# data61/gossamer

Measured on AMD Instinct MI355X. Metric: M k-mers/s (canonical, counted) at k=25, 150 bp reads, higher is better.
Workload: dtype u64

## Files before the change

### gossamer_amd/csrc/fused_path.hpp

```cpp
#pragma once

enum { kFusedDeclined = 0, kFusedDone = 1, kFusedNeedFull = 2, kFusedGoOn = -1, kFusedAgain = -2 };
constexpr uint32_t kFusedGrid = 256 * GOSS_E1_OCC;
#ifndef GOSS_FUSED_NKEYS2
#define GOSS_FUSED_NKEYS2 14
#endif
#ifndef GOSS_FUSED_GRID2
#define GOSS_FUSED_GRID2 512
#endif
constexpr uint32_t kFusedGrid2 = GOSS_FUSED_GRID2;
constexpr double kValidSlackA = 1.06, kValidSlackB = 1.17;
constexpr uint64_t kValidSizingMin = 640u << 20;

struct FusedForm {
    enum Table {
        kSmall,
        kBig,
        kWide,
        k96,
        kRem32
    };
    Table table = kSmall;
    uint32_t segbits = kSegBits;
    bool msd = false;
// ... 497 lines not shown
    if (n == 0) return kFusedDeclined;
    if (n > ch.ka_slots || n > ch.kb_slots) return ch.decline("more keys than the buffers hold");
    const bool narrow = form.rem32() && form.narrow;
    uint64_t tiles = 0, sum = 0;
    const uint64_t tile_keys = narrow ? (uint64_t)(form.r32_bits == 9 ? Sub32N<9>::kTileSlots : Sub32N<10>::kTileSlots)
                             : form.rem32() ? (uint64_t)kSub32Tile : form.msd ? (uint64_t)SubCfg<K>::kTile : (uint64_t)SortCfg<K, false>::kTile;
    for (int d = 0; d < 256; ++d)
    {
        gt->cnt[d] = hp->cursors[d * kCursorStride];
        gt->tile_first[d] = tiles;
        tiles += (gt->cnt[d] + tile_keys - 1) / tile_keys;
        sum += gt->cnt[d];
    }
    gt->tile_first[256] = tiles;
    const uint64_t n_slots = narrow ? n / 3 * 2 : n;
    const uint64_t B = 1ULL << br.blk_log2;
    if (sum < n_slots || sum > n_slots + 8 + (uint64_t)br.grid * 256 * (2 * B + 8))
        throw StatusError{GOSS_ERR_HIP, "fused extraction: bucket counts do not add up"};
    HIP_TRY(hipMemcpyAsync(dgt, gt, sizeof(GapTable), hipMemcpyHostToDevice, c->stream));
    out->n = n; out->tiles = tiles; out->windows = hp->windows;
    return kFusedGoOn;
}

struct FusedLookback { LookbackCtl* ctl; LookbackCtl* hctl; };

inline int count_rem32(const FusedChunk<Key1>& ch, FusedForm form, const Sub32Regions& sub, const FirstLevelResult& fl, const GapTable* dgt,
                       FusedLookback lb, Run* r)
{
    goss_gpu_ctx* c = ch.c;
    Key1* ka = ch.ka; Key1* kb = ch.kb;
    const uint64_t n = fl.n, tiles = fl.tiles;
    const uint32_t r32_regions = form.r32_regions(), r32_bits = form.r32_bits, r32_split = form.r32_split, rbits32 = form.rbits32;
    const uint32_t sqbit32 = c->len - 1;
    const bool narrow = form.narrow, squeeze = form.squeeze;
    SubTable32* dsub = (SubTable32*)c->arena.temp(sizeof(SubTable32));
    unsigned long long* cur2 = (unsigned long long*)c->arena.temp((uint64_t)r32_regions * 4);
    uint64_t* seg_beg = (uint64_t*)c->arena.temp((uint64_t)r32_regions * 8);
    uint64_t* seg_end = (uint64_t*)c->arena.temp((uint64_t)r32_regions * 8);
    Tile32* tdesc = (Tile32*)c->arena.temp(std::max<uint64_t>(tiles, 1) * sizeof(Tile32));
    HIP_TRY(hipMemcpyAsync(dsub->start, sub.start.data(), (uint64_t)r32_regions * 8, hipMemcpyHostToDevice, c->stream));
    HIP_TRY(hipMemcpyAsync(dsub->cap, sub.cap.data(), (uint64_t)r32_regions * 4, hipMemcpyHostToDevice, c->stream));
    HIP_TRY(hipMemsetAsync(cur2, 0, (uint64_t)r32_regions * 4, c->stream));
    if (narrow && r32_bits == 9)
        hipLaunchKernelGGL(HIP_KERNEL_NAME(tiles32_kernel<Sub32N<9>::kTileSlots>), dim3(grid_for(tiles, 256)), dim3(256), 0, c->stream,
                           dgt, tdesc, (uint32_t)tiles);
    else if (narrow)
        hipLaunchKernelGGL(HIP_KERNEL_NAME(tiles32_kernel<Sub32N<10>::kTileSlots>), dim3(grid_for(tiles, 256)), dim3(256), 0, c->stream,
                           dgt, tdesc, (uint32_t)tiles);
    else
        hipLaunchKernelGGL(HIP_KERNEL_NAME(tiles32_kernel<kSub32Tile>), dim3(grid_for(tiles, 256)), dim3(256), 0, c->stream,
                           dgt, tdesc, (uint32_t)tiles);
    {
        PhaseTimer t(c, GOSS_T_SCATTER, n);
        const dim3 g2((uint32_t)((tiles + 7) / 8 * 8));
#define GOSS_LAUNCH_S32N(SQ, B2, NRW)                                                                                    \
    hipLaunchKernelGGL(HIP_KERNEL_NAME(subpart32_kernel<SQ, B2, NRW>), g2, dim3(kTB), 0, c->stream, (const Key1*)ka, (uint32_t*)kb, rbits32, \
                       sqbit32, cur2, (const Tile32*)tdesc, (uint32_t)tiles, (const SubTable32*)dsub, lb.ctl)
#define GOSS_LAUNCH_S32(SQ, B2) do { if (narrow) GOSS_LAUNCH_S32N(SQ, B2, true); else GOSS_LAUNCH_S32N(SQ, B2, false); } while (0)
        if (squeeze) GOSS_LAUNCH_S32(true, 9);
        else if (r32_bits == 9) GOSS_LAUNCH_S32(false, 9);
        else GOSS_LAUNCH_S32(false, 10);
#undef GOSS_LAUNCH_S32
#undef GOSS_LAUNCH_S32N
        t.stop();
    }
    hipLaunchKernelGGL(sub_bounds32_kernel, dim3(r32_regions / 256), dim3(256), 0, c->stream, (const SubTable32*)dsub,
                       (const uint32_t*)cur2, r32_regions, seg_beg, seg_end);
    HIP_TRY(hipMemcpyAsync(lb.hctl, lb.ctl, sizeof(LookbackCtl), hipMemcpyDeviceToHost, c->stream));
    HIP_TRY(hipStreamSynchronize(c->stream));
    if (lb.hctl->error) { c->fused_overflows++; return ch.decline("a 32-bit sub-region overflowed"); }
    ch.lap("second level (32-bit remainders)");
    const uint32_t* rems = (const uint32_t*)kb;
    Key1* spare32 = ka;
    uint32_t nseg32 = r32_regions;
    if (r32_split)
    {
        nseg32 = r32_regions << r32_split;
        uint64_t* sub_beg = (uint64_t*)c->arena.temp((uint64_t)nseg32 * 8);
        uint64_t* sub_end = (uint64_t*)c->arena.temp((uint64_t)nseg32 * 8);
        {
            PhaseTimer t(c, GOSS_T_SCATTER, n);
            hipLaunchKernelGGL(subsplit32_kernel, unit_grid(r32_regions), dim3(kTB), 0, c->stream, (const uint32_t*)kb, (uint32_t*)ka,
                               (const uint64_t*)seg_beg, (const uint64_t*)seg_end, rbits32 - (squeeze ? 1u : 0u), r32_split, sub_beg, sub_end);
            t.stop();
        }
        check_launch("third-level split kernel");
        seg_beg = sub_beg; seg_end = sub_end;
        rems = (const uint32_t*)ka;
        spare32 = kb;
        ch.lap("third level (sub-segments)");
    }
    int rc;
    for (;;)
    {
        rc = segment_reduce32(c, rems, spare32, n, r, seg_beg, seg_end, form.r32_slots, squeeze, rbits32, sqbit32, nseg32, r32_split);
        if (rc != 1 || form.r32_slots >= 16384 || c->rem32_slots) break;
        c->segment_retries++;
        form = form.larger_r32_table();
    }
    if (rc != 0)
    {
        c->segment_retries++;
        if (rc == 1 && r32_split < (uint32_t)kSub32SplitMax) c->rem32_split_min = r32_split + 1;
        else c->rem32 = false;
        if (c->debug) std::fprintf(stderr, "libgossgpu: fused path: 32-bit form with %u + %u bits overflowed (%d), redoing the chunk %s\n", r32_bits, r32_split, rc,
                                   c->rem32 ? "with more sub-segments" : "in the 8-byte form");
        return kFusedAgain;
// ... 241 lines not shown
```

### gossamer_amd/csrc/goss_gpu.hip

```cpp
#include "../../include/goss_gpu.h"

#include <hip/hip_runtime.h>
#include <dlfcn.h>

#include <algorithm>
#include <chrono>
#include <cmath>
#include <cstdio>
#include <cstdlib>
#include <cstring>
#include <functional>
#include <map>
#include <mutex>
#include <string>
#include <system_error>
#include <thread>
#include <vector>

#include "goss_kernels.hpp"
#include "goss_reader.hpp"

using namespace goss;

namespace {
// ... 66 lines not shown
    double est_scale = 1.0;
    uint32_t order_bits = 0;
    bool ordered_tiles = false;
    uint32_t lookback_failures = 0;
    uint64_t emit_estimate = 0;
    bool has_emit_estimate = false;
    struct Pending { hipEvent_t ev; void (*fn)(void*); void* user; };
    std::vector<Pending> pending;
    uint64_t flush_wait_us = 0, flush_count_us = 0, flushes = 0;
    struct PackedSrc { bool on = false; const uint32_t* codes = nullptr; const uint16_t* bad = nullptr; } pk;
    bool stage_pk[2] = {false, false};
    uint8_t* stage_buf[2] = {nullptr, nullptr};
    int stage_cur = 0;
    hipStream_t copy_stream = nullptr;
    std::thread bg;
    int bg_status = GOSS_OK;
    std::string bg_error;
    std::vector<hipEvent_t> pend_pool;
    uint8_t* stage = nullptr;
    uint64_t stage_cap = 0, stage_fill = 0;
    bool mute_timing = false;
    uint32_t segment_retries = 0;
    uint32_t extract_hist_shift = 0xFFFFFFFFu;
    bool extract_rep = false;
    uint32_t rep_chunks = 0;
    bool graph_rep = true;
    int canon_l1 = 1;
    bool more_follows = false;
    uint64_t more_starts = 0;
    uint64_t expect_bases = 0;
    int space_choice = -1;
    uint32_t canon_chunks = 0;
    bool fused = true;
    uint64_t fused_min = 32u << 20;
    uint32_t fused_overflows = 0;
    uint32_t valid_sized_chunks = 0;
    uint32_t valid_resizes = 0;
    uint64_t dump_lo = 0;
    bool dump_live = false;
    uint64_t budget_limit = 0;
    uint32_t arena_grows = 0;
    uint64_t arena_ms = 0;
    std::thread arena_thread;
    int arena_status = GOSS_OK;
    std::string arena_error;
    uint32_t seg_merges = 0;
    uint32_t hash_merges = 0;
    uint64_t hash_merge_min = 1u << 20;
    bool fused_msd = true;
    uint32_t fused_msd_chunks = 0;
    bool rem32 = true;
    int rem32_slots = 0;
    uint32_t narrow_capg = 656;
    bool narrow = true;
    uint32_t r32_small_max = 0;
    bool overflow_by_sort = true;
    uint64_t overflow_units = 0;
    uint32_t rem32_chunks = 0;
    uint32_t narrow_chunks = 0;
    uint64_t assemble_us = 0;
    uint64_t ds_blocks_ranges = 0, ds_blocks_own = 0;
    uint32_t pk_fused_chunks = 0;
    uint32_t pk_unpacked_chunks = 0;
    uint32_t rem32_bits_min = 0;
    uint32_t rem32_bits_last = 0;
    uint32_t rem32_split_min = 0;
    uint32_t rem32_split_last = 0;
    uint32_t fused_chunks = 0;
    bool debug = false;
    double fused_capscale = 1.0;
    uint32_t blk_log2_max = 0;
    bool no_fast32 = false;
    bool table96 = true;
    uint32_t table96_chunks = 0;
    bool wide_table = true;
    bool big_table = true;
    int big_rounds_min = 0;
    uint32_t big_table_chunks = 0;
    uint32_t wide_table_chunks = 0;
    bool rec_mode = false;
    uint32_t rec_chunks = 0;
    bool deferred = false;
    uint8_t* grp_send = nullptr;
    uint64_t grp_send_cap = 0;
    uint8_t* grp_inbox = nullptr;
    uint64_t grp_inbox_cap = 0;
    hipStream_t xstream = nullptr;
    double valid_frac = 1.0;
    bool size_by_valid = true;
    uint64_t budget = 0;
    hipStream_t stream = nullptr;
    bool own_stream = false;
    std::string last_error;
    Arena arena;
    std::vector<Run> runs;
    std::vector<BigMap> big_maps;
    BigMap res_big;
    uint64_t windows = 0, keys_total = 0;
    bool finished = false, emitted = false;
    bool broken = false;
    double grp_count_ms = 0;
    void* res_keys = nullptr;
    uint32_t* res_counts = nullptr;
    uint64_t M = 0;
    void* tips_keys = nullptr;
    uint32_t* tips_counts = nullptr;
// ... 2274 lines not shown
    {
        case GOSS_OK: return "ok";
        case GOSS_ERR_INVALID_ARG: return "invalid argument";
        case GOSS_ERR_NO_DEVICE: return "no usable gfx950 HIP device";
        case GOSS_ERR_OOM: return "out of memory (HBM budget)";
        case GOSS_ERR_HIP: return "HIP runtime error";
        case GOSS_ERR_STATE: return "call out of order";
        case GOSS_ERR_K_RANGE: return "unable to build a graph with that k";
        case GOSS_ERR_COUNT_OVERFLOW: return "a key count does not fit 32 bits";
        case GOSS_ERR_TOO_LARGE: return "SparseArray high bits do not fit 64 bits";
        case GOSS_ERR_BUFFER: return "a buffer of the caller is too small";
        default: return "unknown status";
    }
}

const char* goss_gpu_last_error(const goss_gpu_ctx* ctx) { return ctx ? ctx->last_error.c_str() : ""; }

uint32_t goss_gpu_abi_version(void) { return kAbiVersion; }

int goss_gpu_create(goss_gpu_ctx** out, int device, uint32_t k, int mode, uint64_t hbm_budget, void* stream)
{
    if (!out) return GOSS_ERR_INVALID_ARG;
    *out = nullptr;
    if (mode != GOSS_MODE_KMER_SET && mode != GOSS_MODE_GRAPH) return GOSS_ERR_INVALID_ARG;
    if (k == 0) return GOSS_ERR_K_RANGE;
    if (mode == GOSS_MODE_KMER_SET && k > 63) return GOSS_ERR_K_RANGE;
    if (mode == GOSS_MODE_GRAPH && k > 62) return GOSS_ERR_K_RANGE;
    int ndev = 0;
    if (hipGetDeviceCount(&ndev) != hipSuccess || ndev <= 0 || device < 0 || device >= ndev) return GOSS_ERR_NO_DEVICE;
    hipDeviceProp_t prop;
    if (hipGetDeviceProperties(&prop, device) != hipSuccess) return GOSS_ERR_NO_DEVICE;
    if (std::strncmp(prop.gcnArchName, "gfx950", 6) != 0) return GOSS_ERR_NO_DEVICE;
    goss_gpu_ctx* c = new (std::nothrow) goss_gpu_ctx();
    if (!c) return GOSS_ERR_OOM;
    c->device = device; c->k = k; c->mode = mode;
    c->len = mode == GOSS_MODE_GRAPH ? k + 1 : k;
    c->words = (2 * c->len <= 62) ? 1 : 2;
    c->budget = hbm_budget;
    { const char* e = std::getenv("GOSS_GPU_NO_LOOKBACK"); if (e && *e == '1') c->lookback = false; }
    { const char* e = std::getenv("GOSS_GPU_ORDERED_TILES"); if (e && *e == '1') c->ordered_tiles = true; }
    { const char* e = std::getenv("GOSS_GPU_EST_SCALE"); if (e && std::atof(e) > 0) c->est_scale = std::atof(e); }
    { const char* e = std::getenv("GOSS_GPU_ORDER_BITS"); if (e && std::atoi(e) >= 16 && std::atoi(e) <= 24) c->order_bits = (uint32_t)std::atoi(e); }
    { const char* e = std::getenv("GOSS_GPU_NO_FUSED"); if (e && *e == '1') c->fused = false; }
    { const char* e = std::getenv("GOSS_GPU_NO_MSD"); if (e && *e == '1') c->fused_msd = false; }
    { const char* e = std::getenv("GOSS_GPU_NO_GRAPH_REP"); if (e && *e && *e != '0') c->graph_rep = false; }
    { const char* e = std::getenv("GOSS_GPU_CANON_L1"); if (e && *e >= '0' && *e <= '2') c->canon_l1 = *e - '0'; }
    { const char* e = std::getenv("GOSS_GPU_NO_REM32"); if (e && *e && *e != '0') c->rem32 = false; }
    { const char* e = std::getenv("GOSS_GPU_REM32_BITS"); if (e && std::atoi(e) >= 9 && std::atoi(e) <= 10) c->rem32_bits_min = (uint32_t)std::atoi(e); }
    { const char* e = std::getenv("GOSS_GPU_REM32_SPLIT"); if (e && std::atoi(e) >= 0 && std::atoi(e) <= 4) c->rem32_split_min = (uint32_t)std::atoi(e); }
    { const char* e = std::getenv("GOSS_GPU_REM32_SLOTS"); if (e && (std::atoi(e) == 2048 || std::atoi(e) == 4096 || std::atoi(e) == 8192 || std::atoi(e) == 16384)) c->rem32_slots = std::atoi(e); }
    { const char* e = std::getenv("GOSS_GPU_NARROW"); if (e) c->narrow = std::atoi(e) != 0; }
    { const char* e = std::getenv("GOSS_GPU_OVERFLOW_BY_SORT"); if (e) c->overflow_by_sort = std::atoi(e) != 0; }
    { const char* e = std::getenv("GOSS_GPU_NARROW_CAPG"); if (e && std::atoi(e) > 0) c->narrow_capg = (uint32_t)std::atoi(e); }
    { const char* e = std::getenv("GOSS_GPU_R32_SMALL_MAX"); if (e) c->r32_small_max = (uint32_t)std::atoi(e); }
    { const char* e = std::getenv("GOSS_GPU_NO_BIG_TABLE"); if (e && *e && *e != '0') c->big_table = false; }
    { const char* e = std::getenv("GOSS_GPU_HASH_MERGE_MIN"); if (e && *e) c->hash_merge_min = std::strtoull(e, nullptr, 10); }
    { const char* e = std::getenv("GOSS_GPU_BLK_LOG2"); if (e && *e) c->blk_log2_max = (uint32_t)std::atoi(e); }
    { const char* e = std::getenv("GOSS_GPU_NO_FAST32"); if (e && *e == '1') c->no_fast32 = true; }
    { const char* e = std::getenv("GOSS_GPU_NO_TABLE96"); if (e && *e && *e != '0') c->table96 = false; }
    { const char* e = std::getenv("GOSS_GPU_NO_WIDE_TABLE"); if (e && *e && *e != '0') c->wide_table = false; }
    { const char* e = std::getenv("GOSS_GPU_BIG_ROUNDS_MIN"); if (e && *e) c->big_rounds_min = std::min(3, std::max(0, std::atoi(e))); }
    { const char* e = std::getenv("GOSS_GPU_NO_VALID_SIZING"); if (e && *e && *e != '0') c->size_by_valid = false; }
    { const char* e = std::getenv("GOSS_GPU_FUSED_MIN"); if (e && *e) c->fused_min = std::strtoull(e, nullptr, 10); }
    { const char* e = std::getenv("GOSS_GPU_FUSED_CAPSCALE"); if (e && *e) c->fused_capscale = std::atof(e); }
    { const char* e = std::getenv("GOSS_GPU_DEBUG"); if (e && *e == '1') c->debug = true; }
    int rc = guarded(c, [&]() {
        if (stream) { c->stream = (hipStream_t)stream; c->own_stream = false; }
        else { HIP_TRY(hipStreamCreateWithFlags(&c->stream, hipStreamNonBlocking)); c->own_stream = true; }
        HIP_TRY(hipMalloc((void**)&c->d_ctr, sizeof(ExtractCounters)));
        HIP_TRY(hipMalloc((void**)&c->d_flags, 16));
        HIP_TRY(hipMemsetAsync(c->d_flags, 0, 16, c->stream));
        HIP_TRY(hipHostMalloc(&c->h_pinned, 256, hipHostMallocDefault));
    });
    if (rc != GOSS_OK) { goss_gpu_destroy(c); return rc == GOSS_ERR_HIP ? GOSS_ERR_NO_DEVICE : rc; }
    *out = c;
    return GOSS_OK;
}

int goss_gpu_prepare(goss_gpu_ctx* c)
{
    if (!c) return GOSS_ERR_INVALID_ARG;
    if (c->arena.base || c->arena_thread.joinable()) return GOSS_OK;
    c->arena_status = GOSS_OK;
    c->arena_thread = std::thread([c]() {
        try
        {
            HIP_TRY(hipSetDevice(c->device));
            map_arena(c);
        }
        catch (const HipError& e) { c->arena_status = GOSS_ERR_HIP; c->arena_error = std::string(e.what) + ": " + hipGetErrorString(e.e); }
        catch (const StatusError& e) { c->arena_status = e.status; c->arena_error = e.msg; }
    });
    return GOSS_OK;
}

void goss_gpu_destroy(goss_gpu_ctx* c)
{
    if (!c) return;
    if (c->arena_thread.joinable()) c->arena_thread.join();
    (void)hipSetDevice(c->device);
    if (c->bg.joinable()) c->bg.join();
    if (c->copy_stream) (void)hipStreamSynchronize(c->copy_stream);
    if (c->stream) (void)hipStreamSynchronize(c->stream);
    for (auto& pd : c->pending) { if (pd.fn) pd.fn(pd.user); (void)hipEventDestroy(pd.ev); }
    for (auto e : c->pend_pool) (void)hipEventDestroy(e);
    for (auto*& b : c->stage_buf) if (b) (void)hipFree(b);
// ... 2523 lines not shown
```

### gossamer_amd/csrc/kernels_count.hpp

```cpp
#pragma once
#include <type_traits>

#include <hip/hip_runtime.h>
#include <stdint.h>

#include "goss_key.hpp"
#include "kernels_partition.hpp"

namespace goss {


constexpr int kSegBits = 16;
constexpr int kSegBitsMax = 24;
constexpr int kSegSlots = 4096;
constexpr int kSegLimit = 3072;
constexpr int kSegSlots2 = 2048;
constexpr int kSegLimit2 = 1536;

template <class K>
__global__ void seg_bounds_kernel(const K* __restrict__ keys, uint64_t n, uint32_t shift, uint32_t nseg,
                                  uint64_t* __restrict__ seg_off)
{
    uint32_t s = blockIdx.x * blockDim.x + threadIdx.x;
    if (s > nseg) return;
// ... 686 lines not shown
                    else if (key != mk && eo < 16u)
                    {
                        const uint32_t slot = 4 * bk + (eo >> 2);
                        const uint32_t old = atomicCAS(&tkey[slot], mk, key);
                        if (old == mk) { atomicAdd(&ndist, 1u); hit = slot; }
                        else if (old == key) hit = slot;
                    }
                    else
                    {
                        if (st == 0) { bk = second_of(f, bk); st = 1; }
                        else bk = (bk + 1) & (NB - 1u);
                        if (++moves > NB) { *vovf = 1; busy = false; pd = 0; }
                    }
                    if (hit != ~0u) { atomicAdd(&tcnt[hit], 1u); busy = false; }
                }
            }
        };
        const bool whole = i0 + (uint32_t)NT * kVec <= nfull && (i0 != 0 || head == 0);
        if (whole)
        {
#pragma unroll
            for (int u = 0; u < kVec; ++u)
            {
                const uint32_t left = four_keys(cur[u], 0xFu, std::true_type{});
                if (__builtin_expect(__ballot(left != 0) != 0, 0)) slow_keys(cur[u], left);
            }
        }
        else
        {
#pragma unroll
            for (int u = 0; u < kVec; ++u)
            {
                const uint32_t i = i0 + (uint32_t)u * NT + tid;
                const uint32_t have = i < nvec ? (n - 4u * i >= 4u ? 4u : n - 4u * i) : 0u;
                uint32_t live = (1u << have) - 1u;
                if (i == 0) live &= ~((1u << head) - 1u);
                const uint32_t left = four_keys(cur[u], live, std::false_type{});
                if (__ballot(left != 0)) slow_keys(cur[u], left);
            }
        }
        GOSS_STAMP(2);
        if (*(lds_vu32)&ndist > (uint32_t)kLimit) *vovf = 1;
        if (*vovf) break;
        GOSS_STAMP(3);
    }
    __syncthreads();
    GOSS_STAMP(4);
    if (ovf)
    {
        if (tid == 0) { atomicOr(&so->overflow, 1u); seg_pos[s] = 0; seg_cnt[s] = kSegOverflowed; }
        return;
    }

    constexpr int kPer = SLOTS / NT;
    constexpr int kBins = SLOTS / 4, kBinsPer = kBins / NT, kBinBits = BB;
    __shared__ uint32_t bins[kBins];
    __shared__ uint32_t sh_scan2[NT / 64 + 1];
    __shared__ uint32_t big;
    unsigned long long ck[kPer];
#pragma unroll
    for (int j = 0; j < kPer; ++j) ck[j] = ((unsigned long long)tcnt[tid * kPer + j] << 32) | tkey[tid * kPer + j];
    for (uint32_t i = tid; i < kBins; i += NT) bins[i] = 0;
    if (tid == 0) big = 0;
    __syncthreads();
    const uint32_t rem_bits = rbits - (SQ ? 1u : 0u);
    const uint32_t bsh = rem_bits > (uint32_t)kBinBits + split_bits ? rem_bits - split_bits - kBinBits : 0;
    uint32_t rnk[kPer];
#pragma unroll
    for (int j = 0; j < kPer; ++j)
        if ((ck[j] >> 32) != 0) rnk[j] = atomicAdd(&bins[((uint32_t)ck[j] >> bsh) & (kBins - 1)], 1u);
    __syncthreads();
    uint32_t bn[kBinsPer], bs[kBinsPer], mine = 0;
#pragma unroll
    for (int q = 0; q < kBinsPer; ++q) { bn[q] = bins[tid * kBinsPer + q]; mine += bn[q]; }
    uint32_t tot_occ;
    uint32_t at = block_excl_scan_n<uint32_t, NT / 64>(mine, sh_scan2, &tot_occ);
    lds_vu32 vbig = (lds_vu32)&big;
#pragma unroll
    for (int q = 0; q < kBinsPer; ++q)
    {
        bs[q] = at; bins[tid * kBinsPer + q] = at; at += bn[q];
        if (bn[q] > 24) *vbig = 1;
    }
    __syncthreads();
#pragma unroll
    for (int j = 0; j < kPer; ++j)
        if ((ck[j] >> 32) != 0)
            tab[bins[((uint32_t)ck[j] >> bsh) & (kBins - 1)] + rnk[j]] = (ck[j] << 32) | (ck[j] >> 32);
    __syncthreads();
    if (!big)
    {
#pragma unroll
        for (int q = 0; q < kBinsPer; ++q)
            for (uint32_t i = 1; i < bn[q]; ++i)
            {
                const unsigned long long kk = tab[bs[q] + i];
                uint32_t j = i;
                while (j > 0 && tab[bs[q] + j - 1] > kk) { tab[bs[q] + j] = tab[bs[q] + j - 1]; --j; }
                tab[bs[q] + j] = kk;
            }
        __syncthreads();
    }
    else
    {
        uint32_t nsort = 512;
        while (nsort < tot_occ) nsort <<= 1;
        for (uint32_t i = tot_occ + tid; i < nsort; i += NT) tab[i] = ~0ULL;
        __syncthreads();
        for (uint32_t k2 = 2; k2 <= nsort; k2 <<= 1)
            for (uint32_t j = k2 >> 1; j > 0; j >>= 1)
            {
                for (uint32_t t = tid; t < nsort / 2; t += NT)
                {
                    const uint32_t i = 2 * t - (t & (j - 1));
                    const uint32_t p = i + j;
                    const bool up = (i & k2) == 0;
                    const unsigned long long a = tab[i], c2 = tab[p];
                    if ((a > c2) == up) { tab[i] = c2; tab[p] = a; }
                }
                __syncthreads();
            }
    }
    GOSS_STAMP(5);
    const uint32_t d = ndist;
    if (tid == 0)
    {
        sh_base = atomicAdd(&so->cursor, (unsigned long long)d);
        if (sh_base + d > so->stage_cap) { atomicOr(&so->overflow, 2u); sh_base = ~0ULL; }
        seg_pos[s] = sh_base;
        seg_cnt[s] = d;
    }
    __syncthreads();
    const uint64_t ob = sh_base;
    if (ob == ~0ULL) return;
    const uint64_t prefix = (uint64_t)(s >> split_bits) << rbits;
    for (uint32_t i = tid; i < d; i += NT)
    {
        const unsigned long long v = tab[i];
        stage_keys[ob + i].lo = prefix | rem32_unpack<SQ>((uint32_t)(v >> 32), sqbit);
        stage_counts[ob + i] = (uint32_t)v;
    }
    GOSS_STAMP(6);
#if defined(GOSS_STAMPS)
    if (tid == 0)
    {
        for (int i = 0; i < 7; ++i) atomicAdd(&so->stamps[i], st_acc[i]);
        atomicAdd(&so->stamps[7], 1ULL);
    }
#endif
#undef GOSS_STAMP
}

constexpr uint32_t kSegLock = 0x80000000u;

template <int NT, int SLOTS>
__device__ __forceinline__ void seg_hash_reduce2_body(const Key2* __restrict__ keys, const uint64_t* __restrict__ seg_off,
                                                      const uint64_t* __restrict__ seg_end, SegOut* __restrict__ so, uint64_t* __restrict__ seg_pos,
                                                      uint64_t* __restrict__ seg_cnt,
                                                      Key2* __restrict__ stage_keys, uint32_t* __restrict__ stage_counts,
                                                      uint32_t rem_bits_all, uint32_t round_bits)
{
    constexpr int kLimit = SLOTS / 4 * 3;
    constexpr bool kPow2 = (SLOTS & (SLOTS - 1)) == 0;
    constexpr int kSlotBits = SLOTS == 2048 ? 11 : SLOTS == 4096 ? 12 : SLOTS == 6144 ? 13 : -1;
    static_assert(kSlotBits > 0 && SLOTS % NT == 0, "table size");
    auto next_slot = [](uint32_t a) { return kPow2 ? ((a + 1) & (uint32_t)(SLOTS - 1)) : (a + 1 == (uint32_t)SLOTS ? 0u : a + 1); };
    __shared__ unsigned long long tlo[SLOTS];
    __shared__ unsigned long long thi[SLOTS];
    __shared__ uint32_t st[SLOTS];
    __shared__ uint32_t ndist;
    __shared__ uint32_t ovf;
    __shared__ unsigned long long sh_base;
    const uint32_t s = unit_block(), tid = threadIdx.x;
    const uint32_t sseg = s >> round_bits, rnd = s & ((1u << round_bits) - 1u);
    const uint32_t rsh = rem_bits_all - round_bits;
    const uint64_t b = seg_off[sseg], e = seg_end[sseg];
    if (b == e)
    {
        if (tid == 0) { seg_pos[s] = 0; seg_cnt[s] = 0; }
        return;
    }
// ... 632 lines not shown
```

### gossamer_amd/csrc/kernels_partition.hpp

```cpp
#pragma once

#include <hip/hip_runtime.h>
#include <stdint.h>

#include "goss_key.hpp"
#include "kernels_common.hpp"

namespace goss {


#ifndef GOSS_SORT_ITEMS1
#define GOSS_SORT_ITEMS1 32
#endif
#ifndef GOSS_SORT_ITEMS2
#define GOSS_SORT_ITEMS2 16
#endif
#ifndef GOSS_LB_BATCH
#define GOSS_LB_BATCH 1
#endif
template <class K> struct SubCfg {
    static constexpr int kItems = sizeof(K) == 8 ? 22 : 11;
    static constexpr int kTile = 256 * kItems;
};

// ... 486 lines not shown

struct Tile32 { unsigned long long base; uint32_t n, bucket; };
#ifndef GOSS_S32_ITEMS
#define GOSS_S32_ITEMS 22
#endif
constexpr int kSub32Items = GOSS_S32_ITEMS;
constexpr int kSub32Tile = kTB * kSub32Items;
template <int TILE>
__global__ void tiles32_kernel(const GapTable* __restrict__ gt, Tile32* __restrict__ desc, uint32_t total)
{
    const uint32_t t = blockIdx.x * blockDim.x + threadIdx.x;
    if (t >= total) return;
    uint32_t lo = 0, hi = 255;
    while (lo < hi)
    {
        const uint32_t mid = (lo + hi + 1) >> 1;
        if (gt->tile_first[mid] <= t) lo = mid; else hi = mid - 1;
    }
    const uint64_t j = (uint64_t)t - gt->tile_first[lo];
    const uint64_t left = gt->cnt[lo] - j * TILE;
    desc[t] = Tile32{gt->reg_start[lo] + j * TILE, (uint32_t)(left < (uint64_t)TILE ? left : (uint64_t)TILE), lo};
}

#ifndef GOSS_S32_OCC
#define GOSS_S32_OCC 4
#endif
#ifndef GOSS_S32_CH
#define GOSS_S32_CH 10
#define GOSS_S32_OCCN 3
#endif
template <int B2> struct Sub32N { static constexpr int kChunks = B2 == 9 ? GOSS_S32_CH : GOSS_S32_CH - 1; static constexpr int kTileSlots = kTB * kChunks * 2; };
template <bool SQ, int B2, bool NARROW = false>
__global__ __launch_bounds__(kTB, NARROW ? GOSS_S32_OCCN : GOSS_S32_OCC) void subpart32_kernel(const Key1* __restrict__ keys_in, uint32_t* __restrict__ out,
                                                           uint32_t rbits, uint32_t sqbit, unsigned long long* __restrict__ cursors,
                                                           const Tile32* __restrict__ desc, uint32_t total_tiles,
                                                           const SubTable32* __restrict__ sub, LookbackCtl* __restrict__ ctl)
{
    constexpr int kSub32ChunksN = Sub32N<B2>::kChunks;
    constexpr int kItems = NARROW ? 3 * kSub32ChunksN : kSub32Items;
    static_assert(NARROW || kItems <= 32, "one bit of `have` per key");
    constexpr int kTile = kTB * kItems;
    constexpr uint32_t ND = 1u << B2;
    constexpr int DPT = ND / kTB;
    static_assert(DPT >= 2 && DPT % 2 == 0, "a thread owns pairs of digits");
    __shared__ uint32_t stage[kTile];
    __shared__ uint16_t sdig[kTile];
    __shared__ uint32_t hist[ND];
    __shared__ uint32_t gbase[ND];
    __shared__ uint32_t sh_scan[kWaves + 1];
    __shared__ uint32_t sh_skip, sh_total;

    const uint32_t tid = threadIdx.x, lane = lane_id(), w = wave_id();
    const uint32_t per = (total_tiles + 7u) / 8u;
    const uint32_t tile = (blockIdx.x & 7u) * per + (blockIdx.x >> 3);
    if (tile >= total_tiles) return;
    const Tile32 td = desc[tile];
    const uint32_t b = td.bucket, tile_n = td.n;
    const uint64_t tile_base = td.base;
    if (tid == 0) sh_skip = 0;
#pragma unroll
    for (int j = 0; j < DPT; ++j) hist[tid + j * kTB] = 0;

    __builtin_amdgcn_s_setprio(3);
    Key1 key[NARROW ? 1 : kItems];
    [[maybe_unused]] uint32_t rem[NARROW ? kItems : 1], dw[NARROW ? kSub32ChunksN : 1];
    uint16_t rank[kItems];
    uint32_t have = 0;
    const uint32_t wbase = w * 64 * kItems;
    if constexpr (NARROW)
    {
        const uint32_t nchunk = tile_n >> 1;
        const uint4* const cin = reinterpret_cast<const uint4*>(keys_in + tile_base);
        const uint32_t cbase = w * 64 * kSub32ChunksN;
#pragma unroll
        for (int r = 0; r < kSub32ChunksN; ++r)
        {
            const uint32_t ci = cbase + r * 64 + lane;
            dw[r] = 0;
            rem[3 * r] = rem[3 * r + 1] = rem[3 * r + 2] = 0;
            if (ci < nchunk)
            {
                const uint4 v = cin[ci];
                rem[3 * r] = v.x; rem[3 * r + 1] = v.y; rem[3 * r + 2] = v.z; dw[r] = v.w;
            }
        }
        __builtin_amdgcn_s_setprio(0);
        __syncthreads();
#pragma unroll
        for (int r = 0; r < kItems; ++r)
            if ((dw[r / 3] >> 30) > (uint32_t)(r % 3)) rank[r] = (uint16_t)atomicAdd(&hist[(dw[r / 3] >> (10 * (r % 3))) & (ND - 1u)], 1u);
    }
    else
    {
#if !defined(GOSS_S32_LOAD8)
    static_assert(kItems % 2 == 0, "pairs of keys per load");
#pragma unroll
    for (int r = 0; r < kItems / 2; ++r)
    {
        const uint32_t li = wbase + r * 128 + 2 * lane;
        if (li < tile_n)
        {
#if defined(GOSS_S32_NT)
            typedef uint32_t u32x4_ __attribute__((ext_vector_type(4)));
            const u32x4_ vv = __builtin_nontemporal_load(reinterpret_cast<const u32x4_*>(keys_in + tile_base + li));
            const uint4 v = make_uint4(vv.x, vv.y, vv.z, vv.w);
#else
            const uint4 v = *reinterpret_cast<const uint4*>(keys_in + tile_base + li);
#endif
            key[2 * r].lo = (uint64_t)v.x | ((uint64_t)v.y << 32);
            key[2 * r + 1].lo = (uint64_t)v.z | ((uint64_t)v.w << 32);
            have |= 3u << (2 * r);
        }
    }
#else
#pragma unroll
    for (int r = 0; r < kItems; ++r)
    {
        const uint32_t li = wbase + r * 64 + lane;
        if (li < tile_n) { key[r] = keys_in[tile_base + li]; have |= 1u << r; }
    }
#endif
    __builtin_amdgcn_s_setprio(0);
    __syncthreads();
#pragma unroll
    for (int r = 0; r < kItems; ++r)
        if (((have >> r) & 1u) && is_pad_key(key[r])) have &= ~(1u << r);
#pragma unroll
    for (int r = 0; r < kItems; ++r)
        if ((have >> r) & 1u) rank[r] = (uint16_t)atomicAdd(&hist[(uint32_t)(key[r].lo >> rbits) & (ND - 1u)], 1u);
    }
    __syncthreads();
    const uint64_t region_first = sub->start[b * ND];
    {
        uint32_t cn[DPT], ex[DPT], mine = 0;
        const uint32_t sidx = b * ND + DPT * tid;
#pragma unroll
        for (int j = 0; j < DPT; ++j) { cn[j] = hist[DPT * tid + j]; mine += cn[j]; }
        bool over = false;
#pragma unroll
        for (int j = 0; j < DPT; j += 2)
        {
            unsigned long long old = 0;
            if (cn[j] | cn[j + 1]) old = atomicAdd(&cursors[(sidx + j) >> 1], (unsigned long long)cn[j] | ((unsigned long long)cn[j + 1] << 32));
            ex[j] = (uint32_t)old; ex[j + 1] = (uint32_t)(old >> 32);
            over |= (cn[j] && ex[j] + cn[j] > sub->cap[sidx + j]) || (cn[j + 1] && ex[j + 1] + cn[j + 1] > sub->cap[sidx + j + 1]);
        }
        if (over) { atomicOr(&ctl->error, 2u); sh_skip = 1; }
        uint32_t tile_total;
        uint32_t start = block_excl_scan<uint32_t>(mine, sh_scan, &tile_total);
#pragma unroll
        for (int j = 0; j < DPT; ++j)
        {
            hist[DPT * tid + j] = start;
            gbase[DPT * tid + j] = (mine ? (uint32_t)(sub->start[sidx + j] - region_first) : 0u) + ex[j] - start;
            start += cn[j];
        }
        if (tid == 0) sh_total = tile_total;
    }
    __syncthreads();
#pragma unroll
    for (int r = 0; r < kItems; ++r)
        if (NARROW ? (dw[NARROW ? r / 3 : 0] >> 30) > (uint32_t)(r % 3) : ((have >> (r & 31)) & 1u) != 0)
        {
            if constexpr (NARROW)
            {
                const uint32_t d = (dw[r / 3] >> (10 * (r % 3))) & (ND - 1u);
                const uint32_t at = hist[d] + rank[r];
                stage[at] = rem[r];
                sdig[at] = (uint16_t)d;
            }
            else
            {
            const uint32_t d = (uint32_t)(key[r].lo >> rbits) & (ND - 1u);
            const uint32_t at = hist[d] + rank[r];
            stage[at] = rem32_pack<SQ>(key[r].lo, rbits, sqbit);
            sdig[at] = (uint16_t)d;
            }
        }
    __syncthreads();
    if (sh_skip) return;
    const uint32_t tile_keys = sh_total;
    uint32_t* const out_r = out + region_first;
    for (uint32_t i = tid; i < tile_keys; i += kTB)
    {
#if defined(GOSS_S32_EXP) && GOSS_S32_EXP == 1
        asm volatile("" ::"v"(gbase[sdig[i]]), "v"(stage[i]));
#else
        out_r[(uint32_t)(gbase[sdig[i]] + i)] = stage[i];
#endif
    }
}

__global__ void sub_bounds32_kernel(const SubTable32* __restrict__ sub, const uint32_t* __restrict__ cursors, uint32_t nseg,
                                    uint64_t* __restrict__ seg_beg, uint64_t* __restrict__ seg_end)
{
    const uint32_t s = blockIdx.x * blockDim.x + threadIdx.x;
    if (s >= nseg) return;
    seg_beg[s] = sub->start[s];
    seg_end[s] = sub->start[s] + cursors[s];
}

__global__ __launch_bounds__(kTB) void subsplit32_kernel(const uint32_t* __restrict__ in, uint32_t* __restrict__ out,
                                                         const uint64_t* __restrict__ seg_beg, const uint64_t* __restrict__ seg_end,
                                                         uint32_t rem_bits, uint32_t b3, uint64_t* __restrict__ sub_beg,
                                                         uint64_t* __restrict__ sub_end)
{
    typedef uint32_t u32x4 __attribute__((ext_vector_type(4)));
    __shared__ uint32_t cnt[kWaves][64][17];
    __shared__ uint32_t wcnt[kWaves][16];
    const uint32_t s = unit_block(), tid = threadIdx.x, lane = lane_id(), w = wave_id();
    const uint32_t nd = 1u << b3, dsh = rem_bits - b3;
    const uint64_t b = seg_beg[s], e = seg_end[s];
    if (b == e)
    {
        if (tid < nd) { sub_beg[(uint64_t)s * nd + tid] = b; sub_end[(uint64_t)s * nd + tid] = b; }
        return;
    }
    for (uint32_t j = 0; j < 17; ++j) cnt[w][lane][j] = 0;
    const uint64_t n = e - b;
    const uint64_t nvec = (n + 3) >> 2;
    const u32x4* const in4 = reinterpret_cast<const u32x4*>(in + b);
    for (uint64_t i = tid; i < nvec; i += kTB)
    {
        const u32x4 v = in4[i];
        const uint32_t kk[4] = {v.x, v.y, v.z, v.w};
#pragma unroll
        for (int j = 0; j < 4; ++j)
            if (4 * i + j < n) cnt[w][lane][(kk[j] >> dsh) & (nd - 1u)] += 1u;
    }
    __syncthreads();
    if (tid < (uint32_t)kWaves * 16u)
    {
        const uint32_t ww = tid >> 4, d = tid & 15u;
        uint32_t sum = 0;
        for (uint32_t l = 0; l < 64; ++l) sum += cnt[ww][l][d];
        wcnt[ww][d] = d < nd ? sum : 0u;
    }
    __syncthreads();
    if (tid == 0)
    {
        uint64_t at = 0;
        for (uint32_t d = 0; d < nd; ++d)
// ... 70 lines not shown
```

Baseline: 179,600.

## Make subpart32 scatter persistent with prefetch of next tile's chunks

The 32-bit sub-partition scatter kernel now runs as a persistent grid capped by occupancy. Each block loops over tiles within its XCD slice and prefetches the next tile's narrow chunks while the current tile's cursor atomics and scan are in flight. Per-tile cursor atomics are issued unconditionally and their cap checks are deferred, and ranks are packed two per register. Separately, the count kernel issues its stage-cursor atomic at kernel start to hide its latency. The cost is higher register pressure from double-buffering, plus extra atomics on zero counts.

```diff
diff --git a/gossamer_amd/csrc/fused_path.hpp b/gossamer_amd/csrc/fused_path.hpp
--- a/gossamer_amd/csrc/fused_path.hpp
+++ b/gossamer_amd/csrc/fused_path.hpp
@@ -573,7 +573,8 @@
                            dgt, tdesc, (uint32_t)tiles);
     {
         PhaseTimer t(c, GOSS_T_SCATTER, n);
-        const dim3 g2((uint32_t)((tiles + 7) / 8 * 8));
+        const uint32_t g2_full = 256u * (narrow ? (uint32_t)GOSS_S32_OCCN : (uint32_t)GOSS_S32_OCC);
+        const dim3 g2(c->s32_grid ? c->s32_grid : (uint32_t)std::min<uint64_t>((std::max<uint64_t>(tiles, 1) + 7) / 8 * 8, g2_full));
 #define GOSS_LAUNCH_S32N(SQ, B2, NRW)                                                                                    \
     hipLaunchKernelGGL(HIP_KERNEL_NAME(subpart32_kernel<SQ, B2, NRW>), g2, dim3(kTB), 0, c->stream, (const Key1*)ka, (uint32_t*)kb, rbits32, \
                        sqbit32, cur2, (const Tile32*)tdesc, (uint32_t)tiles, (const SubTable32*)dsub, lb.ctl)
diff --git a/gossamer_amd/csrc/goss_gpu.hip b/gossamer_amd/csrc/goss_gpu.hip
--- a/gossamer_amd/csrc/goss_gpu.hip
+++ b/gossamer_amd/csrc/goss_gpu.hip
@@ -142,6 +142,7 @@
     bool rem32 = true;
     int rem32_slots = 0;
     uint32_t narrow_capg = 656;
+    uint32_t s32_grid = 0;
     bool narrow = true;
     uint32_t r32_small_max = 0;
     bool overflow_by_sort = true;
@@ -2522,6 +2523,7 @@
     { const char* e = std::getenv("GOSS_GPU_NARROW"); if (e) c->narrow = std::atoi(e) != 0; }
     { const char* e = std::getenv("GOSS_GPU_OVERFLOW_BY_SORT"); if (e) c->overflow_by_sort = std::atoi(e) != 0; }
     { const char* e = std::getenv("GOSS_GPU_NARROW_CAPG"); if (e && std::atoi(e) > 0) c->narrow_capg = (uint32_t)std::atoi(e); }
+    { const char* e = std::getenv("GOSS_GPU_S32_GRID"); if (e && std::atoi(e) >= 8 && std::atoi(e) <= 65536 && std::atoi(e) % 8 == 0) c->s32_grid = (uint32_t)std::atoi(e); }
     { const char* e = std::getenv("GOSS_GPU_R32_SMALL_MAX"); if (e) c->r32_small_max = (uint32_t)std::atoi(e); }
     { const char* e = std::getenv("GOSS_GPU_NO_BIG_TABLE"); if (e && *e && *e != '0') c->big_table = false; }
     { const char* e = std::getenv("GOSS_GPU_HASH_MERGE_MIN"); if (e && *e) c->hash_merge_min = std::strtoull(e, nullptr, 10); }
diff --git a/gossamer_amd/csrc/kernels_count.hpp b/gossamer_amd/csrc/kernels_count.hpp
--- a/gossamer_amd/csrc/kernels_count.hpp
+++ b/gossamer_amd/csrc/kernels_count.hpp
@@ -762,6 +762,14 @@
         return;
     }
 
+    const uint32_t d = ndist;
+    unsigned long long cursor_old = 0, stage_cap = 0;
+    if (tid == 0)
+    {
+        cursor_old = atomicAdd(&so->cursor, (unsigned long long)d);
+        stage_cap = so->stage_cap;
+    }
+
     constexpr int kPer = SLOTS / NT;
     constexpr int kBins = SLOTS / 4, kBinsPer = kBins / NT, kBinBits = BB;
     __shared__ uint32_t bins[kBins];
@@ -832,11 +840,10 @@
             }
     }
     GOSS_STAMP(5);
-    const uint32_t d = ndist;
     if (tid == 0)
     {
-        sh_base = atomicAdd(&so->cursor, (unsigned long long)d);
-        if (sh_base + d > so->stage_cap) { atomicOr(&so->overflow, 2u); sh_base = ~0ULL; }
+        sh_base = cursor_old;
+        if (sh_base + d > stage_cap) { atomicOr(&so->overflow, 2u); sh_base = ~0ULL; }
         seg_pos[s] = sh_base;
         seg_cnt[s] = d;
     }
diff --git a/gossamer_amd/csrc/kernels_partition.hpp b/gossamer_amd/csrc/kernels_partition.hpp
--- a/gossamer_amd/csrc/kernels_partition.hpp
+++ b/gossamer_amd/csrc/kernels_partition.hpp
@@ -562,142 +562,199 @@
 
     const uint32_t tid = threadIdx.x, lane = lane_id(), w = wave_id();
     const uint32_t per = (total_tiles + 7u) / 8u;
-    const uint32_t tile = (blockIdx.x & 7u) * per + (blockIdx.x >> 3);
-    if (tile >= total_tiles) return;
-    const Tile32 td = desc[tile];
-    const uint32_t b = td.bucket, tile_n = td.n;
-    const uint64_t tile_base = td.base;
-    if (tid == 0) sh_skip = 0;
+    const uint32_t xcd_first = (blockIdx.x & 7u) * per, tstep = gridDim.x >> 3;
+    uint32_t tj = blockIdx.x >> 3;
+    if (tj >= per || xcd_first + tj >= total_tiles) return;
+    Tile32 td = desc[xcd_first + tj];
 #pragma unroll
     for (int j = 0; j < DPT; ++j) hist[tid + j * kTB] = 0;
 
-    __builtin_amdgcn_s_setprio(3);
     Key1 key[NARROW ? 1 : kItems];
     [[maybe_unused]] uint32_t rem[NARROW ? kItems : 1], dw[NARROW ? kSub32ChunksN : 1];
-    uint16_t rank[kItems];
-    uint32_t have = 0;
-    const uint32_t wbase = w * 64 * kItems;
+    [[maybe_unused]] uint32_t nrem[NARROW ? kItems : 1], ndw[NARROW ? kSub32ChunksN : 1];
+    uint32_t rank2[(kItems + 1) / 2] = {};
+    auto set_rank = [&](int r, uint32_t v) { rank2[r / 2] = (r & 1) ? (rank2[r / 2] & 0xFFFFu) | (v << 16) : v; };
+    auto get_rank = [&](int r) { return (r & 1) ? rank2[r / 2] >> 16 : rank2[r / 2] & 0xFFFFu; };
+    [[maybe_unused]] const uint32_t wbase = w * 64 * kItems;
+    [[maybe_unused]] const uint32_t cbase = w * 64 * kSub32ChunksN + lane;
+    [[maybe_unused]] auto load_chunks = [&](const Tile32& t, uint32_t (&rm)[NARROW ? kItems : 1], uint32_t (&d)[NARROW ? kSub32ChunksN : 1]) {
+        const uint32_t nchunk = t.n >> 1;
+        const uint32_t last = nchunk ? nchunk - 1u : 0u;
+        const uint4* const cin = reinterpret_cast<const uint4*>(keys_in + t.base);
+#pragma unroll
+        for (int r = 0; r < kSub32ChunksN; ++r)
+        {
+            const uint32_t ci = cbase + r * 64;
+            const uint4 v = cin[ci < last ? ci : last];
+            rm[3 * r] = v.x; rm[3 * r + 1] = v.y; rm[3 * r + 2] = v.z; d[r] = v.w;
+        }
+    };
     if constexpr (NARROW)
     {
-        const uint32_t nchunk = tile_n >> 1;
-        const uint4* const cin = reinterpret_cast<const uint4*>(keys_in + tile_base);
-        const uint32_t cbase = w * 64 * kSub32ChunksN;
-#pragma unroll
-        for (int r = 0; r < kSub32ChunksN; ++r)
-        {
-            const uint32_t ci = cbase + r * 64 + lane;
-            dw[r] = 0;
-            rem[3 * r] = rem[3 * r + 1] = rem[3 * r + 2] = 0;
-            if (ci < nchunk)
-            {
-                const uint4 v = cin[ci];
-                rem[3 * r] = v.x; rem[3 * r + 1] = v.y; rem[3 * r + 2] = v.z; dw[r] = v.w;
-            }
-        }
+        __builtin_amdgcn_s_setprio(3);
+        load_chunks(td, rem, dw);
         __builtin_amdgcn_s_setprio(0);
+#pragma unroll
+        for (int r = 0; r < kSub32ChunksN; ++r) asm volatile("" ::"v"(rem[3 * r]), "v"(rem[3 * r + 1]), "v"(rem[3 * r + 2]), "v"(dw[r]));
+    }
+
+    for (;;)
+    {
+        const uint32_t tj_next = tj + tstep;
+        const bool more = tj_next < per && xcd_first + tj_next < total_tiles;
+        Tile32 tn = td;
+        if (more) tn = desc[xcd_first + tj_next];
+        const uint32_t b = td.bucket;
+        [[maybe_unused]] uint32_t have = 0;
+        if constexpr (!NARROW)
+        {
+            const uint32_t tile_n = td.n;
+            const uint64_t tile_base = td.base;
+            __builtin_amdgcn_s_setprio(3);
+#if !defined(GOSS_S32_LOAD8)
+            static_assert(kItems % 2 == 0, "pairs of keys per load");
+#pragma unroll
+            for (int r = 0; r < kItems / 2; ++r)
+            {
+                const uint32_t li = wbase + r * 128 + 2 * lane;
+                if (li < tile_n)
+                {
+#if defined(GOSS_S32_NT)
+                    typedef uint32_t u32x4_ __attribute__((ext_vector_type(4)));
+                    const u32x4_ vv = __builtin_nontemporal_load(reinterpret_cast<const u32x4_*>(keys_in + tile_base + li));
+                    const uint4 v = make_uint4(vv.x, vv.y, vv.z, vv.w);
+#else
+                    const uint4 v = *reinterpret_cast<const uint4*>(keys_in + tile_base + li);
+#endif
+                    key[2 * r].lo = (uint64_t)v.x | ((uint64_t)v.y << 32);
+                    key[2 * r + 1].lo = (uint64_t)v.z | ((uint64_t)v.w << 32);
+                    have |= 3u << (2 * r);
+                }
+            }
+#else
+#pragma unroll
+            for (int r = 0; r < kItems; ++r)
+            {
+                const uint32_t li = wbase + r * 64 + lane;
+                if (li < tile_n) { key[r] = keys_in[tile_base + li]; have |= 1u << r; }
+            }
+#endif
+            __builtin_amdgcn_s_setprio(0);
+        }
         __syncthreads();
+        if (tid == 0) sh_skip = 0;
+        if constexpr (NARROW)
+        {
+            const uint32_t nchunk = td.n >> 1;
+#pragma unroll
+            for (int r = 0; r < kSub32ChunksN; ++r)
+                if (cbase + r * 64 >= nchunk) dw[r] = 0;
+#pragma unroll
+            for (int r = 0; r < kItems; ++r)
+                if ((dw[r / 3] >> 30) > (uint32_t)(r % 3)) set_rank(r, atomicAdd(&hist[(dw[r / 3] >> (10 * (r % 3))) & (ND - 1u)], 1u));
+        }
+        else
+        {
+#pragma unroll
+            for (int r = 0; r < kItems; ++r)
+                if (((have >> r) & 1u) && is_pad_key(key[r])) have &= ~(1u << r);
+#pragma unroll
+            for (int r = 0; r < kItems; ++r)
+                if ((have >> r) & 1u) set_rank(r, atomicAdd(&hist[(uint32_t)(key[r].lo >> rbits) & (ND - 1u)], 1u));
+        }
+        __syncthreads();
+        const uint64_t region_first = sub->start[b * ND];
+        uint32_t cn[DPT], cap[DPT], mine = 0;
+        unsigned long long old[DPT / 2];
+        uint32_t sstart[DPT];
+        const uint32_t sidx = b * ND + DPT * tid;
+#pragma unroll
+        for (int j = 0; j < DPT; ++j) { cn[j] = hist[DPT * tid + j]; mine += cn[j]; }
+        if constexpr (NARROW)
+        {
+            __builtin_amdgcn_s_setprio(3);
+            load_chunks(tn, nrem, ndw);
+            __builtin_amdgcn_s_setprio(0);
+        }
+#pragma unroll
+        for (int j = 0; j < DPT; j += 2)
+        {
+            old[j / 2] = atomicAdd(&cursors[(sidx + j) >> 1], (unsigned long long)cn[j] | ((unsigned long long)cn[j + 1] << 32));
+        }
+#pragma unroll
+        for (int j = 0; j < DPT; ++j) { cap[j] = sub->cap[sidx + j]; sstart[j] = reinterpret_cast<const uint32_t*>(&sub->start[sidx + j])[0]; }
+        uint32_t tile_total;
+        const uint32_t start0 = block_excl_scan<uint32_t>(mine, sh_scan, &tile_total);
+        {
+            uint32_t start = start0;
+#pragma unroll
+            for (int j = 0; j < DPT; ++j) { hist[DPT * tid + j] = start; start += cn[j]; }
+        }
+        if (tid == 0) sh_total = tile_total;
+        __syncthreads();
 #pragma unroll
         for (int r = 0; r < kItems; ++r)
-            if ((dw[r / 3] >> 30) > (uint32_t)(r % 3)) rank[r] = (uint16_t)atomicAdd(&hist[(dw[r / 3] >> (10 * (r % 3))) & (ND - 1u)], 1u);
-    }
-    else
-    {
-#if !defined(GOSS_S32_LOAD8)
-    static_assert(kItems % 2 == 0, "pairs of keys per load");
-#pragma unroll
-    for (int r = 0; r < kItems / 2; ++r)
-    {
-        const uint32_t li = wbase + r * 128 + 2 * lane;
-        if (li < tile_n)
-        {
-#if defined(GOSS_S32_NT)
-            typedef uint32_t u32x4_ __attribute__((ext_vector_type(4)));
-            const u32x4_ vv = __builtin_nontemporal_load(reinterpret_cast<const u32x4_*>(keys_in + tile_base + li));
-            const uint4 v = make_uint4(vv.x, vv.y, vv.z, vv.w);
+            if (NARROW ? (dw[NARROW ? r / 3 : 0] >> 30) > (uint32_t)(r % 3) : ((have >> (r & 31)) & 1u) != 0)
+            {
+                if constexpr (NARROW)
+                {
+                    const uint32_t d = (dw[r / 3] >> (10 * (r % 3))) & (ND - 1u);
+                    const uint32_t at = hist[d] + get_rank(r);
+                    stage[at] = rem[r];
+                    sdig[at] = (uint16_t)d;
+                }
+                else
+                {
+                    const uint32_t d = (uint32_t)(key[r].lo >> rbits) & (ND - 1u);
+                    const uint32_t at = hist[d] + get_rank(r);
+                    stage[at] = rem32_pack<SQ>(key[r].lo, rbits, sqbit);
+                    sdig[at] = (uint16_t)d;
+                }
+            }
+        {
+            bool over = false;
+            uint32_t start = start0;
+#pragma unroll
+            for (int j = 0; j < DPT; ++j)
+            {
+                const uint32_t ex = (uint32_t)(old[j / 2] >> (32 * (j & 1)));
+                over |= cn[j] && ex + cn[j] > cap[j];
+                gbase[DPT * tid + j] = sstart[j] - (uint32_t)region_first + ex - start;
+                start += cn[j];
+            }
+            if (over) { atomicOr(&ctl->error, 2u); sh_skip = 1; }
+        }
+        __syncthreads();
+        const bool skip = sh_skip != 0;
+        const uint32_t tile_keys = sh_total;
+#pragma unroll
+        for (int j = 0; j < DPT; ++j) hist[tid + j * kTB] = 0;
+        if constexpr (NARROW)
+        {
+#pragma unroll
+            for (int r = 0; r < kSub32ChunksN; ++r) asm volatile("" ::"v"(nrem[3 * r]), "v"(nrem[3 * r + 1]), "v"(nrem[3 * r + 2]), "v"(ndw[r]));
+        }
+        if (!skip)
+        {
+            uint32_t* const out_r = out + region_first;
+            for (uint32_t i = tid; i < tile_keys; i += kTB)
+            {
+#if defined(GOSS_S32_EXP) && GOSS_S32_EXP == 1
+                asm volatile("" ::"v"(gbase[sdig[i]]), "v"(stage[i]));
 #else
-            const uint4 v = *reinterpret_cast<const uint4*>(keys_in + tile_base + li);
-#endif
-            key[2 * r].lo = (uint64_t)v.x | ((uint64_t)v.y << 32);
-            key[2 * r + 1].lo = (uint64_t)v.z | ((uint64_t)v.w << 32);
-            have |= 3u << (2 * r);
-        }
-    }
-#else
-#pragma unroll
-    for (int r = 0; r < kItems; ++r)
-    {
-        const uint32_t li = wbase + r * 64 + lane;
-        if (li < tile_n) { key[r] = keys_in[tile_base + li]; have |= 1u << r; }
-    }
-#endif
-    __builtin_amdgcn_s_setprio(0);
-    __syncthreads();
-#pragma unroll
-    for (int r = 0; r < kItems; ++r)
-        if (((have >> r) & 1u) && is_pad_key(key[r])) have &= ~(1u << r);
-#pragma unroll
-    for (int r = 0; r < kItems; ++r)
-        if ((have >> r) & 1u) rank[r] = (uint16_t)atomicAdd(&hist[(uint32_t)(key[r].lo >> rbits) & (ND - 1u)], 1u);
-    }
-    __syncthreads();
-    const uint64_t region_first = sub->start[b * ND];
-    {
-        uint32_t cn[DPT], ex[DPT], mine = 0;
-        const uint32_t sidx = b * ND + DPT * tid;
-#pragma unroll
-        for (int j = 0; j < DPT; ++j) { cn[j] = hist[DPT * tid + j]; mine += cn[j]; }
-        bool over = false;
-#pragma unroll
-        for (int j = 0; j < DPT; j += 2)
-        {
-            unsigned long long old = 0;
-            if (cn[j] | cn[j + 1]) old = atomicAdd(&cursors[(sidx + j) >> 1], (unsigned long long)cn[j] | ((unsigned long long)cn[j + 1] << 32));
-            ex[j] = (uint32_t)old; ex[j + 1] = (uint32_t)(old >> 32);
-            over |= (cn[j] && ex[j] + cn[j] > sub->cap[sidx + j]) || (cn[j + 1] && ex[j + 1] + cn[j + 1] > sub->cap[sidx + j + 1]);
-        }
-        if (over) { atomicOr(&ctl->error, 2u); sh_skip = 1; }
-        uint32_t tile_total;
-        uint32_t start = block_excl_scan<uint32_t>(mine, sh_scan, &tile_total);
-#pragma unroll
-        for (int j = 0; j < DPT; ++j)
-        {
-            hist[DPT * tid + j] = start;
-            gbase[DPT * tid + j] = (mine ? (uint32_t)(sub->start[sidx + j] - region_first) : 0u) + ex[j] - start;
-            start += cn[j];
-        }
-        if (tid == 0) sh_total = tile_total;
-    }
-    __syncthreads();
-#pragma unroll
-    for (int r = 0; r < kItems; ++r)
-        if (NARROW ? (dw[NARROW ? r / 3 : 0] >> 30) > (uint32_t)(r % 3) : ((have >> (r & 31)) & 1u) != 0)
-        {
-            if constexpr (NARROW)
-            {
-                const uint32_t d = (dw[r / 3] >> (10 * (r % 3))) & (ND - 1u);
-                const uint32_t at = hist[d] + rank[r];
-                stage[at] = rem[r];
-                sdig[at] = (uint16_t)d;
-            }
-            else
-            {
-            const uint32_t d = (uint32_t)(key[r].lo >> rbits) & (ND - 1u);
-            const uint32_t at = hist[d] + rank[r];
-            stage[at] = rem32_pack<SQ>(key[r].lo, rbits, sqbit);
-            sdig[at] = (uint16_t)d;
-            }
-        }
-    __syncthreads();
-    if (sh_skip) return;
-    const uint32_t tile_keys = sh_total;
-    uint32_t* const out_r = out + region_first;
-    for (uint32_t i = tid; i < tile_keys; i += kTB)
-    {
-#if defined(GOSS_S32_EXP) && GOSS_S32_EXP == 1
-        asm volatile("" ::"v"(gbase[sdig[i]]), "v"(stage[i]));
-#else
-        out_r[(uint32_t)(gbase[sdig[i]] + i)] = stage[i];
-#endif
+                out_r[(uint32_t)(gbase[sdig[i]] + i)] = stage[i];
+#endif
+            }
+        }
+        if (!more) break;
+        td = tn; tj = tj_next;
+        if constexpr (NARROW)
+        {
+#pragma unroll
+            for (int r = 0; r < kItems; ++r) rem[r] = nrem[r];
+#pragma unroll
+            for (int r = 0; r < kSub32ChunksN; ++r) dw[r] = ndw[r];
+        }
     }
 }
 
```

After: 171,400. 0.954x the previous value.
